# sarpaykent/GotenNet

Measured on AMD Instinct MI355X. Metric: molecules/sec (energy+force forward), rMD17 aspirin batch=128, 1/2/4/8 MI355X, higher is better.
Workload: dtype f32 (2xfp16-split MFMA with block exponents, fp32 accumulate); 1 GPU; rmd17_aspirin batch=128/GPU (N=2688 atoms, E=54368 edges incl. self-loops), n_atom_basis=256, n_interactions=6, lmax=2, n_rbf=32, heads=8, sep_dir/sep_tensor, energy+forces; global_batch=128, parallelism=dp1 (molecule shards, 1 all-reduce)

## Files before the change

gotennet_amd/csrc/gn_backward.hip:

```cpp
#include "gn_common.h"
#include "gn_tune.h"
#include "gn_sh.h"
#include "gn_highl.h"

namespace gn {


template <int K>
__device__ __forceinline__ void slot_sums(const float (&v)[K], int lps, int lp, float* __restrict__ arr, size_t base) {
    constexpr int KP = K <= 4 ? 4 : (K <= 8 ? 8 : (K <= 16 ? 16 : 32));
    if (lps >= KP) {
        float vals[KP];
#pragma unroll
        for (int k = 0; k < KP; ++k) vals[k] = k < K ? v[k] : 0.f;
        multi_group_sum<KP>(vals, lps, lp);
        const int stride = lps / KP;
        if ((lp & (stride - 1)) == 0 && lp / stride < K) arr[base + lp / stride] = vals[0];
    } else {
#pragma unroll
        for (int k = 0; k < K; ++k) {
            const float s = group_sum(v[k], lps);
            if (lp == 0) arr[base + k] = s;
        }
    }
}

template <int MS>
__device__ __forceinline__ void slot_head_sums(const float* hrow, int lps, int lp, int H, float* __restrict__ out) {
    const int rpl = lps / H, hh = lp / rpl, part = lp - hh * rpl;
    const float* hp = hrow + hh * (MS * rpl) + part * MS;
    float hv = hp[0];
#pragma unroll
    for (int k = 1; k < MS; ++k) hv += hp[k];
    hv = group_sum(hv, rpl);
    if (part == 0) out[hh] = hv;
}

constexpr int GS_CAP = 2048;
template <bool GS_LDS>
struct HeadGrads {
    float* gsl; float* g_s; int e0, H;
    __device__ __forceinline__ float& operator()(int e, int h) const {
        if constexpr (GS_LDS) return gsl[(e - e0) * H + h];
        else return g_s[(size_t)e * H + h];
    }
    __device__ __forceinline__ void copy_out(int e1) const {
        if constexpr (GS_LDS) {
            const int n = (e1 - e0) * H;
            for (int idx = threadIdx.x; idx < n; idx += 256) g_s[(size_t)e0 * H + idx] = gsl[idx];
        }
    }
};
template <typename Grads>
__device__ __forceinline__ void softmax_bwd_head(int e0, int e1, int H, int h, float dot, const float* __restrict__ a,
                                                 const float* __restrict__ a_soft, const int* __restrict__ outdeg,
                                                 const int* __restrict__ src, float inv_sqrt_f, Grads GS) {
    for (int e = e0 + (threadIdx.x & 63); e < e1; e += 64) {
        const float nrm = outdeg ? sqrtf((float)outdeg[src[e]]) * inv_sqrt_f : inv_sqrt_f;
        const float av = a[(size_t)e * H + h];
        const float sv = a_soft ? a_soft[(size_t)e * H + h] : av;
        GS(e, h) = av * GS(e, h) - (sv / nrm) * dot;
    }
}
__device__ __forceinline__ void score_bwd_edge(float gs, float4 qi, float4 kj, float4 pta, float4& gq, float* __restrict__ g_pta) {
    float4 a_ta, d_ta;
    act_pair4(pta, GN_ACT_SILU, a_ta, d_ta);
    gq = fma4(gs, kj * a_ta, gq);
    st4_nt(g_pta, ((qi * kj) * gs) * d_ta);
}
__device__ __forceinline__ float4 score_bwd_edge_k(float gs, float4 qi, float4 pta, float4 gk) {
    return fma4(gs, qi * act4(pta, GN_ACT_SILU), gk);
}

template <int LMAX, int FC = 0>
__global__ __launch_bounds__(256) GN_WPE(GN_W_HTR_SRC) void htr_bwd_source_kernel(
    const float* __restrict__ gtp, const float* __restrict__ pre_t,
    const float* __restrict__ EQ, const float* __restrict__ EK, const float* __restrict__ rl,
    const int* __restrict__ colptr, const int* __restrict__ perm, const int* __restrict__ dst, int N, int F_rt,
    float* __restrict__ gEK) {
    constexpr int act = GN_ACT_SILU;
    constexpr int D = (LMAX + 1) * (LMAX + 1) - 1;
    constexpr int CH = D < 9 ? D : 9;
    __shared__ __attribute__((aligned(16))) float red[CH * 1024];
    const int F = FC ? FC : F_rt;
    const int j = xcd_item(blockIdx.x, N);
    if (j < 0) return;
    GN_SLOT_GEOMETRY(FC);
    const int p0 = colptr[j], p1 = colptr[j + 1];
    float4 ek[D], acc[D];
#pragma unroll
    for (int m = 0; m < D; ++m) { ek[m] = ld4(EK + ((size_t)j * D + m) * F + c0); acc[m] = zero4(); }
    for (int pp = p0 + slot; pp < p1; pp += ns) {
        const int e = perm[pp];
        const float4 gw = ld4(gtp + (size_t)e * F + c0) * act4(ld4(pre_t + (size_t)e * F + c0), act);
        const float* qi = EQ + (size_t)dst[pp] * D * F + c0;
        const float* re = rl + (size_t)e * D;
        int m0 = 0;
#pragma unroll
        for (int l = 1; l <= LMAX; ++l) {
            float4 eq[2 * LMAX + 1];
            float r[2 * LMAX + 1];
            float4 pa = zero4();
            float rr = 0.f;
#pragma unroll
            for (int mm = 0; mm < 2 * l + 1; ++mm) {
                eq[mm] = ld4(qi + (size_t)(m0 + mm) * F);
                r[mm] = re[m0 + mm];
                pa = fma4(r[mm], eq[mm], pa);
                rr = fmaf(r[mm], r[mm], rr);
            }
            const float4 v = gw * pa * (rr - 2.0f);
#pragma unroll
            for (int mm = 0; mm < 2 * l + 1; ++mm)
                acc[m0 + mm] = fma4(r[mm], v, fma4(gw, eq[mm], acc[m0 + mm]));
            m0 += 2 * l + 1;
        }
    }
    reduce_rows<D>(acc, red, slot, c0, F, ns, [&](int row, float4 s) { st4(gEK + ((size_t)j * D + row) * F + c0, s); });
}

template <int LMAX, bool SEP_DIR, bool SEP_TENSOR>
struct MsgShape {
    static constexpr int D = (LMAX + 1) * (LMAX + 1) - 1;
    static constexpr int ND = SEP_DIR ? LMAX : 1;
    static constexpr int NT = SEP_TENSOR ? LMAX : 1;
    static constexpr int M = 1 + ND + NT;
    __host__ __device__ static constexpr bool is_dir(int b) { return b >= 1 && b < 1 + ND; }
    __host__ __device__ static constexpr int lo(int b) { return is_dir(b) ? (SEP_DIR ? b : 1) : (SEP_TENSOR ? b - ND : 1); }
    __host__ __device__ static constexpr int hi(int b) { return is_dir(b) ? (SEP_DIR ? b : LMAX) : (SEP_TENSOR ? b - ND : LMAX); }
    __host__ __device__ static constexpr int first_row(int l) { return l * l - 1; }
};


template <int LMAX, bool SEP_DIR, bool SEP_TENSOR, bool GS_LDS, bool FIRST, int FC>
__device__ __forceinline__ void msg_bwd_target_body(const MsgBwdArgs& p, float* gsl, float* red, float* hsum, const float* __restrict__ x_, const float* __restrict__ v_, const float* __restrict__ eproj_, const float* __restrict__ a_, const float* __restrict__ qk_, const float* __restrict__ X_in_, const float* __restrict__ rl_, const float* __restrict__ cut_, const int* __restrict__ outdeg_, const float* __restrict__ g_h1_, const float* __restrict__ g_X1_, const int* __restrict__ rowptr_, const int* __restrict__ src_, float* __restrict__ g_eproj_, float* __restrict__ g_s_, float* __restrict__ g_nproj_, float* __restrict__ g_rl_, float* __restrict__ g_cut_) {
    using S = MsgShape<LMAX, SEP_DIR, SEP_TENSOR>;
    constexpr int D = S::D, M = S::M;
    const int N = p.N, F = FC ? FC : p.F, H = p.H;
    const int i = xcd_item(blockIdx.x, N);
    if (i < 0) return;
    GN_SLOT_GEOMETRY(FC);
    const int e0 = rowptr_[i], e1 = rowptr_[i + 1];
    const int per_head = (M * F) / H;
    int hb[M];
// ... 293 lines not shown
        if (row < MB) st4(g_x + (size_t)j * ldxv + row * F + c0, sv);
        else if (row < 2 * MB) st4(g_v + (size_t)j * ldxv + (row - MB) * F + c0, sv);
        else {
            const size_t off = ((size_t)j * D + (row - 2 * MB)) * F + c0;
            st4(g_X_out + off, ld4(g_X1 + off) + sv);
        }
    });
    if (FIRST)
        for (int b = MB + slot; b < M; b += ns) {
            st4(g_x + (size_t)j * ldxv + b * F + c0, zero4());
            st4(g_v + (size_t)j * ldxv + b * F + c0, zero4());
        }
}
#define GN_MSGB_SOURCE_PTRS(p)                                                                                        \
    p.x, p.v, p.ldxv, p.X_in, p.eproj, p.lde, p.a, p.rl, p.cut, p.g_h1, p.g_X1, p.dst, p.colptr, p.perm, p.g_eproj, p.g_x, p.g_v, \
        p.g_X_out, p.g_rl
template <int LMAX, bool SEP_DIR, bool SEP_TENSOR, int FC = 0>
__global__ __launch_bounds__(256) GN_WPE(GN_W_MSG_MRG) void msg_bwd_merged_kernel(const MsgBwdArgs p, float* __restrict__ ga) {
    msg_bwd_merged_body<LMAX, SEP_DIR, SEP_TENSOR, FC, false>(GN_MSGB_SOURCE_PTRS(p), p.g_cut, ga, p.N, p.F, p.H);
}
template <int LMAX, bool SEP_DIR, bool SEP_TENSOR, int FC = 0>
__global__ __launch_bounds__(256) GN_WPE(GN_W_MSG_MRG_F) void msg_bwd_merged_first_kernel(const MsgBwdArgs p, float* __restrict__ ga) {
    msg_bwd_merged_body<LMAX, SEP_DIR, SEP_TENSOR, FC, true>(GN_MSGB_SOURCE_PTRS(p), p.g_cut, ga, p.N, p.F, p.H);
}

template <int FC = 0>
__global__ __launch_bounds__(256) void msg_bwd_gk_kernel(const MsgBwdArgs p) {
    __shared__ __attribute__((aligned(16))) float red[1024];
    const int N = p.N, F = FC ? FC : p.F, H = p.H;
    const int j = xcd_item(blockIdx.x, N);
    if (j < 0) return;
    GN_SLOT_GEOMETRY(FC);
    const int hq = c0 / (F / H);
    float4 gk[1] = {zero4()};
    for (int pp = p.colptr[j] + slot; pp < p.colptr[j + 1]; pp += ns) {
        const int e = p.perm[pp], i = p.dst[pp];
        gk[0] = score_bwd_edge_k(p.g_s[(size_t)e * H + hq], ld4(p.qk + (size_t)i * p.ldqk + c0),
                                 ld4_nt(p.eproj + (size_t)e * p.lde + c0), gk[0]);
    }
    reduce_rows<1>(gk, red, slot, c0, F, ns, [&](int, float4 sv) { st4(p.g_nproj + (size_t)j * p.ldn + F + c0, sv); });
}

template <bool GS_LDS, int FC>
__device__ __forceinline__ void attn_bwd_body(const MsgBwdArgs& p, const float* __restrict__ ga_parts, int G, size_t gstride,
                                              float* red, float* gsl, int i) {
    const int F = FC ? FC : p.F, H = p.H;
    GN_SLOT_GEOMETRY(FC);
    const int e0 = p.rowptr[i], e1 = p.rowptr[i + 1];
    const HeadGrads<GS_LDS> GS{gsl, p.g_s, e0, H};
    {
        const int wave = threadIdx.x >> 6, lane = threadIdx.x & 63;
        for (int h = wave; h < H; h += 4) {
            float dot = 0.f;
            for (int e = e0 + lane; e < e1; e += 64) {
                float ga = 0.f;
                for (int q = 0; q < G; ++q) ga += ga_parts[q * gstride + (size_t)e * H + h];
                GS(e, h) = ga;
                dot += p.a[(size_t)e * H + h] * ga;
            }
            softmax_bwd_head(e0, e1, H, h, wave_sum(dot), p.a, p.a_soft, p.outdeg, p.src, p.inv_sqrt_f, GS);
        }
    }
    __syncthreads();
    GS.copy_out(e1);
    const int hq = c0 / (F / H);
    const float4 qi = ld4(p.qk + (size_t)i * p.ldqk + c0);
    float4 gq = zero4();
    for (int e = e0 + slot; e < e1; e += ns) {
        const float4 kj = ld4(p.qk + (size_t)p.src[e] * p.ldqk + F + c0);
        score_bwd_edge(GS(e, hq), qi, kj, ld4_nt(p.eproj + (size_t)e * p.lde + c0), gq, p.g_eproj + (size_t)e * p.lde + c0);
    }
    st4(&red[slot * F + c0], gq);
    __syncthreads();
    if (slot == 0) st4(p.g_nproj + (size_t)i * p.ldn + c0, red4(red, c0, F, ns));
}
template <int FC = 0>
__global__ __launch_bounds__(256) void attn_bwd_kernel(const MsgBwdArgs p, const float* __restrict__ ga_parts, int G, size_t gstride) {
    __shared__ __attribute__((aligned(16))) float red[1024];
    __shared__ float gsl[GS_CAP];
    const int i = xcd_item(blockIdx.x, p.N);
    if (i < 0) return;
    if ((p.rowptr[i + 1] - p.rowptr[i]) * p.H <= GS_CAP) attn_bwd_body<true, FC>(p, ga_parts, G, gstride, red, gsl, i);
    else attn_bwd_body<false, FC>(p, ga_parts, G, gstride, red, gsl, i);
}

template <int LMAX, int LLO, int LHI, bool SCALAR, int FC>
__device__ __forceinline__ void msg_bwd_merged_group_body(
    const float* __restrict__ x, const float* __restrict__ v, int ldxv, const float* __restrict__ X_in,
    const float* __restrict__ eproj, int lde, const float* __restrict__ a, const float* __restrict__ rl,
    const float* __restrict__ cut, const float* __restrict__ g_h1, const float* __restrict__ g_X1,
    const int* __restrict__ dst, const int* __restrict__ colptr, const int* __restrict__ perm,
    float* __restrict__ g_eproj, float* __restrict__ g_x, float* __restrict__ g_v, float* __restrict__ g_X_out,
    float* __restrict__ g_rl, float* __restrict__ ga_slice, float* __restrict__ cut_slice, int N, int F_rt, int H) {
    constexpr int D = (LMAX + 1) * (LMAX + 1) - 1;
    constexpr int M = 1 + 2 * LMAX;
    constexpr int NL = LHI - LLO + 1;
    constexpr int XR = (LHI + 1) * (LHI + 1) - LLO * LLO, M0 = LLO * LLO - 1;
    constexpr int NB = (SCALAR ? 1 : 0) + 2 * NL;
    constexpr int ROWS = 2 * NB + XR;
    constexpr int CH = ROWS < 9 ? ROWS : 9;
    constexpr int KP = (XR + 8) <= 16 ? 16 : 32;
    __shared__ __attribute__((aligned(16))) float red[CH * 1024];
    __shared__ __attribute__((aligned(16))) float own[ROWS * 256];
    const int F = FC ? FC : F_rt;
    const int j = xcd_item(blockIdx.x, N);
    if (j < 0) return;
    GN_SLOT_GEOMETRY(FC);
    const int p0 = colptr[j], p1 = colptr[j + 1];
    const int per_head = (M * F) / H;
    auto vblock = [&](int k) { return SCALAR ? (k == 0 ? 0 : (k <= NL ? LLO + k - 1 : LMAX + LLO + k - 1 - NL))
                                             : (k < NL ? LLO + k : LMAX + LLO + k - NL); };
    for (int idx = threadIdx.x * 4; idx < ROWS * F; idx += 1024) {
        const int r = idx / F, c = idx - r * F;
        const float* g = r < NB ? x + (size_t)j * ldxv + vblock(r) * F
                                : (r < 2 * NB ? v + (size_t)j * ldxv + vblock(r - NB) * F
                                              : X_in + ((size_t)j * D + M0 + (r - 2 * NB)) * F);
        st4(own + idx, ld4(g + c));
    }
    float4 acc[ROWS];
#pragma unroll
    for (int r = 0; r < ROWS; ++r) acc[r] = zero4();
    __syncthreads();

    int pp = p0 + slot;
    int e_n = 0, i_n = 0;
    if (pp < p1) { e_n = perm[pp]; i_n = dst[pp]; }
    for (; pp < p1; pp += ns) {
        const int e = e_n, i = i_n;
        if (pp + ns < p1) { e_n = perm[pp + ns]; i_n = dst[pp + ns]; }
        const float* tr = eproj + (size_t)e * lde + F + c0;
        float* gtr = g_eproj + (size_t)e * lde + F + c0;
        const float* ar = a + (size_t)e * H;
        const float* re = rl + (size_t)e * D;
        const float* gXi = g_X1 + (size_t)i * D * F + c0;
        int oc = c0;
        asm volatile("" : "+v"(oc));
        const float* ox = own + oc;
        const float* ov = own + NB * F + oc;
        const float* oX = own + 2 * NB * F + oc;
        float4 tf[NB], gxa[XR];
        float ab_[NB];
#pragma unroll
        for (int k = 0; k < NB; ++k) tf[k] = ld4_nt(tr + vblock(k) * F);
#pragma unroll
        for (int m = 0; m < XR; ++m) gxa[m] = ld4(gXi + (size_t)(M0 + m) * F);
        float4 gh = zero4();
        if (SCALAR) gh = ld4(g_h1 + (size_t)i * F + c0);
        const float ce = cut[e];
#pragma unroll
        for (int k = 0; k < NB; ++k) ab_[k] = ar[(vblock(k) * F + c0) / per_head];
        float cutp = 0.f;
        float vals[KP];
#pragma unroll
        for (int k = 0; k < KP; ++k) vals[k] = 0.f;
        auto block = [&](int b, int k, float4 go) {
            const float4 tfb = tf[k], xb = ld4(ox + k * F), vb = ld4(ov + k * F);
            const int hb = (b * F + c0) / per_head;
            const float ab = ab_[k];
            st4_nt(gtr + b * F, (go * xb) * ce);
            cutp += hsum4(go * tfb * xb);
            const float pa = hsum4(go * vb);
#pragma unroll
            for (int h = 0; h < 8; ++h) vals[XR + h] += (hb == h) ? pa : 0.f;
            acc[k] = fma4(go, tfb * ce, acc[k]);
            acc[NB + k] = fma4(ab, go, acc[NB + k]);
            return fma4(ab, vb, (tfb * xb) * ce);
// ... 431 lines not shown
        for (int n = n0 + lane; n < n1; n += 64) s += y[n];
        s = wave_sum(s);
        if (lane == 0) energy[b] = ((mean && n1 > n0) ? s / (float)(n1 - n0) : s) + mol_shift;
    }
    if (atom_scale)
        for (int n = n0 + (int)threadIdx.x; n < n1; n += 1024) atom_scale[n] = mean ? 1.0f / (float)(n1 - n0) : 1.0f;
}

__global__ void head_grad_kernel(const float* __restrict__ pre1, const float* __restrict__ W2, float scale,
                                 const float* __restrict__ atom_scale, int N, int Hd, float* __restrict__ gpre1, int act) {
    const size_t idx = (size_t)blockIdx.x * blockDim.x + threadIdx.x;
    if (idx >= (size_t)N * Hd) return;
    const float sc = atom_scale ? scale * atom_scale[idx / Hd] : scale;
    gpre1[idx] = sc * W2[idx % Hd] * dact1(pre1[idx], act);
}

}

static bool bwd_dim_ok_wide(int F) { return F >= 16 && F <= 1024 && gn::is_pow2(F); }

#define GN_SWITCH_LMAX(KERNEL, grid, block, st, ...)                                                   \
    switch (lmax) {                                                                                    \
        case 1: hipLaunchKernelGGL(gn::KERNEL<1>, grid, block, 0, st, __VA_ARGS__); break;             \
        case 2: hipLaunchKernelGGL(gn::KERNEL<2>, grid, block, 0, st, __VA_ARGS__); break;             \
        case 3: hipLaunchKernelGGL(gn::KERNEL<3>, grid, block, 0, st, __VA_ARGS__); break;             \
        case 4: hipLaunchKernelGGL(gn::KERNEL<4>, grid, block, 0, st, __VA_ARGS__); break;             \
        case 5: hipLaunchKernelGGL(gn::KERNEL<5>, grid, block, 0, st, __VA_ARGS__); break;             \
        case 6: hipLaunchKernelGGL(gn::KERNEL<6>, grid, block, 0, st, __VA_ARGS__); break;             \
        case 7: hipLaunchKernelGGL(gn::KERNEL<7>, grid, block, 0, st, __VA_ARGS__); break;             \
        default: hipLaunchKernelGGL(gn::KERNEL<8>, grid, block, 0, st, __VA_ARGS__); break;            \
    }

template <int FC>
static void htr_backward_launch(const float* g_t_out, const float* pre_t, const float* w, const float* EQ, const float* EK,
                                const float* rl, const int* rowptr, const int* src, const int* dst, const int* colptr,
                                const int* perm, int N, int F, int lmax, float* gEQ, float* gEK, float* g_rl, float* g_pre_t,
                                hipStream_t st) {
    const dim3 grid(gn::xcd_grid(N)), block(256);
#define GN_HTRB_T(L, LLO, LHI, FIRST)                                                                            \
    hipLaunchKernelGGL((gn::htr_bwd_target_group_kernel<L, LLO, LHI, FIRST, FC>), grid, block, 0, st, g_t_out, pre_t, w, \
                       EQ, EK, rl, rowptr, src, N, F, gEQ, g_rl, g_pre_t)
#define GN_HTRB_S(...)                                                                                           \
    hipLaunchKernelGGL((gn::__VA_ARGS__), grid, block, 0, st, g_t_out, pre_t, EQ, EK, rl, colptr, perm, dst, N, F, gEK)
    switch (lmax) {
        case 1: GN_HTRB_T(1, 1, 1, true); GN_HTRB_S(htr_bwd_source_kernel<1, FC>); break;
        case 2: GN_HTRB_T(2, 1, 2, true); GN_HTRB_S(htr_bwd_source_kernel<2, FC>); break;
        case 3: GN_HTRB_T(3, 1, 3, true); GN_HTRB_S(htr_bwd_source_group_kernel<3, 1, 3, FC>); break;
        default: GN_HTRB_T(4, 1, 2, true); GN_HTRB_T(4, 3, 4, false); GN_HTRB_S(htr_bwd_source_group_kernel<4, 1, 4, FC>); break;
    }
#undef GN_HTRB_T
#undef GN_HTRB_S
}

extern "C" int gn_htr_backward(const float* g_t_out, const float* pre_t, const float* w, const float* w_raw,
                               const float* EQ,
                               const float* EK, const float* rl, const int* rowptr, const int* src, const int* dst,
                               const int* colptr, const int* perm, int N, int F, int lmax_arg, int mode,
                               float* gEQ, float* gEK, float* g_rl, float* g_pre_t, int act, void* stream) {
    const int lmax = lmax_arg & 0xff;
    if ((lmax_arg & ~(0xff | GN_LMAX_SLICED)) || !bwd_dim_ok_wide(F) || N < 0 || lmax < 1 || lmax > 8 || mode < 0 || mode > 31 ||
        act < 0 || act >= GN_ACT_COUNT)
        return GN_ERR_BAD_ARG;
    if (N == 0) return GN_OK;
    hipStream_t st = (hipStream_t)stream;
    if (gn_use_highl(lmax_arg) || F > 256 || (!mode && act != GN_ACT_SILU))
        return gn_highl_htr_backward(g_t_out, pre_t, w, w_raw, EQ, EK, rl, rowptr, src, dst, colptr, perm, N, F, lmax,
                                     mode, gEQ, gEK, g_rl, g_pre_t, act, st);
    if (mode)
        return gn_htr_backward_general(g_t_out, pre_t, w, w_raw, EQ, EK, rl, rowptr, src, dst, colptr, perm, N, F, lmax,
                                       mode, gEQ, gEK, g_rl, g_pre_t, act, st);
    if (F == 256) htr_backward_launch<256>(g_t_out, pre_t, w, EQ, EK, rl, rowptr, src, dst, colptr, perm, N, F, lmax, gEQ, gEK, g_rl, g_pre_t, st);
    else htr_backward_launch<0>(g_t_out, pre_t, w, EQ, EK, rl, rowptr, src, dst, colptr, perm, N, F, lmax, gEQ, gEK, g_rl, g_pre_t, st);
    GN_LAUNCH_CHECK();
    return GN_OK;
}

template <int L, int LLO, int LHI, bool SC, int FC>
static inline void gn_launch_msg_bwd_group(dim3 grid, dim3 block, hipStream_t st, const gn::MsgBwdArgs& p, float* ga_slice, float* cut_slice) {
    if constexpr (LLO == 3 && LHI == 3)
        hipLaunchKernelGGL((gn::msg_bwd_merged_group3_kernel<L, LLO, LHI, SC, FC>), grid, block, 0, st, p, ga_slice, cut_slice);
    else
        hipLaunchKernelGGL((gn::msg_bwd_merged_group_kernel<L, LLO, LHI, SC, FC>), grid, block, 0, st, p, ga_slice, cut_slice);
}
template <int L, bool SD, bool ST, int FC>
static void gn_launch_msg_bwd(dim3 grid, dim3 block, hipStream_t st, const gn::MsgBwdArgs& p, float* ga_parts) {
    constexpr bool GROUPED = L >= 3 && SD && ST;
    if (ga_parts != nullptr) {
        if (!p.X_in) hipLaunchKernelGGL((gn::msg_bwd_merged_first_kernel<L, SD, ST, FC>), grid, block, 0, st, p, ga_parts);
        else if constexpr (!GROUPED) hipLaunchKernelGGL((gn::msg_bwd_merged_kernel<L, SD, ST, FC>), grid, block, 0, st, p, ga_parts);
        hipLaunchKernelGGL(gn::attn_bwd_kernel<FC>, grid, block, 0, st, p, ga_parts, 1, (size_t)0);
        hipLaunchKernelGGL(gn::msg_bwd_gk_kernel<FC>, grid, block, 0, st, p);
    } else if (!p.X_in) {
        hipLaunchKernelGGL((gn::msg_bwd_target_kernel<L, SD, ST, true, FC>), grid, block, 0, st, p);
        hipLaunchKernelGGL((gn::msg_bwd_source_kernel<L, SD, ST, true, FC>), grid, block, 0, st, p);
    } else if constexpr (!GROUPED) {
        hipLaunchKernelGGL((gn::msg_bwd_target_kernel<L, SD, ST>), grid, block, 0, st, p);
        hipLaunchKernelGGL((gn::msg_bwd_source_kernel<L, SD, ST>), grid, block, 0, st, p);
    }
}

extern "C" int gn_message_backward_groups(int lmax_arg, int sep_dir, int sep_tensor, int act) {
    const int lmax = lmax_arg & 0xff;
    if (gn_use_highl(lmax_arg) || act != GN_ACT_SILU) return 1;
    return (lmax >= 3 && sep_dir && sep_tensor) ? lmax - 1 : 1;
}

template <int FC>
static void message_backward_launch(const gn::MsgBwdArgs& p, int lmax, int sep_dir, int sep_tensor, bool groups, float* ga_parts,
                                    long E, hipStream_t st) {
    const dim3 grid(gn::xcd_grid(p.N)), block(256);
    if (groups) {
        const size_t gs = (size_t)E * p.H;
#define GN_MSGB_M(L, LLO, LHI, SC, G)                                                                        \
    gn_launch_msg_bwd_group<L, LLO, LHI, SC, FC>(grid, block, st, p, ga_parts + (size_t)(G) * gs, p.g_cut + (size_t)(G) * E)
        if (lmax == 3) { GN_MSGB_M(3, 1, 2, true, 0); GN_MSGB_M(3, 3, 3, false, 1); }
        else { GN_MSGB_M(4, 1, 2, true, 0); GN_MSGB_M(4, 3, 3, false, 1); GN_MSGB_M(4, 4, 4, false, 2); }
#undef GN_MSGB_M
        hipLaunchKernelGGL(gn::attn_bwd_kernel<FC>, grid, block, 0, st, p, ga_parts, lmax - 1, gs);
        hipLaunchKernelGGL(gn::msg_bwd_gk_kernel<FC>, grid, block, 0, st, p);
        return;
    }
#define GN_MSGB_CASE(L, SD, ST, W) \
    case (L) * 4 + (SD ? 2 : 0) + (ST ? 1 : 0): gn_launch_msg_bwd<L, SD, ST, W>(grid, block, st, p, ga_parts); break
    switch (lmax * 4 + (sep_dir ? 2 : 0) + (sep_tensor ? 1 : 0)) {
        case 4: case 5: case 6: case 7:
            gn_launch_msg_bwd<1, false, false, FC>(grid, block, st, p, ga_parts);
            break;
        GN_MSGB_CASE(2, false, false, 0);
        GN_MSGB_CASE(2, false, true, 0);
        GN_MSGB_CASE(2, true, false, 0);
        GN_MSGB_CASE(2, true, true, FC);
        GN_MSGB_CASE(3, false, false, 0);
        GN_MSGB_CASE(3, false, true, 0);
        GN_MSGB_CASE(3, true, false, 0);
        GN_MSGB_CASE(3, true, true, FC);
        GN_MSGB_CASE(4, false, false, 0);
        GN_MSGB_CASE(4, false, true, 0);
        GN_MSGB_CASE(4, true, false, 0);
        default: gn_launch_msg_bwd<4, true, true, FC>(grid, block, st, p, ga_parts); break;
    }
#undef GN_MSGB_CASE
}

static int message_backward(
    const float* x, const float* v, int ldxv, const float* eproj, int lde, const float* a,
    const float* qk, int ldqk, const float* X_in, const float* rl, const float* cut, const int* outdeg,
    const float* g_h1, const float* g_X1,
    const int* rowptr, const int* src, const int* dst, const int* colptr, const int* perm,
    float* g_eproj, float* g_s, float* g_nproj, int ldn, float* g_x, float* g_v, float* g_X_out,
    float* g_rl, float* g_cut, float* ga_parts, long E,
    int N, int F, int H, int lmax_arg, int sep_dir, int sep_tensor, int act, void* stream, const float* a_soft) {
    const int lmax = lmax_arg & 0xff;
    const bool amax = (lmax_arg & GN_LMAX_MAX) != 0;
    if (amax && ((lmax_arg & GN_LMAX_MEAN) || !ga_parts || !X_in)) return GN_ERR_BAD_ARG;
    if ((lmax_arg & ~(0xff | GN_LMAX_SLICED | GN_LMAX_MEAN | GN_LMAX_MAX)) || !bwd_dim_ok_wide(F) || N < 0 || H <= 0 || !gn::is_pow2(H) || (F / 4) % H || (F / 4) / H > 64 || lmax < 1 || lmax > 8 ||
        (ldxv & 3) || (lde & 3) || (ldqk & 3) || (ldn & 3) || g_X_out == g_X1 || act < 0 || act >= GN_ACT_COUNT)
        return GN_ERR_BAD_ARG;
    if (!X_in && (act != GN_ACT_SILU || gn_use_highl(lmax_arg) || F > 256)) return GN_ERR_BAD_ARG;
    if (N == 0) return GN_OK;
    gn::MsgBwdArgs p{x, v, ldxv, eproj, lde, a, qk, ldqk, X_in, rl, cut, outdeg, g_h1, g_X1,
                     rowptr, src, dst, colptr, perm, g_eproj, g_s, g_nproj, ldn, g_x, g_v, g_X_out, g_rl, g_cut,
                     N, F, H, (float)(1.0 / sqrt((double)F)), act, (lmax_arg & GN_LMAX_MEAN) ? 1 : 0, amax ? ga_parts : nullptr, a_soft};
    hipStream_t st = (hipStream_t)stream;
    if (gn_use_highl(lmax_arg) || F > 256 || act != GN_ACT_SILU) return gn_highl_message_backward(p, lmax, sep_dir, sep_tensor, st);
    const int G = gn_message_backward_groups(lmax_arg, sep_dir, sep_tensor, act);
    const bool groups = X_in && G > 1;
    if (groups && (ga_parts == nullptr || E <= 0)) return GN_ERR_BAD_ARG;
    if (groups && H > 8) {
        hipError_t err = hipMemsetAsync(g_cut + E, 0, (size_t)(G - 1) * (size_t)E * sizeof(float), st);
        if (err != hipSuccess) return (int)err;
        return gn_highl_message_backward(p, lmax, sep_dir, sep_tensor, st);
    }
    if (F == 256) message_backward_launch<256>(p, lmax, sep_dir, sep_tensor, groups, ga_parts, E, st);
    else message_backward_launch<0>(p, lmax, sep_dir, sep_tensor, groups, ga_parts, E, st);
    GN_LAUNCH_CHECK();
    return GN_OK;
}

extern "C" int gn_message_backward(
    const float* x, const float* v, int ldxv, const float* eproj, int lde, const float* a,
    const float* qk, int ldqk, const float* X_in, const float* rl, const float* cut, const int* outdeg,
    const float* g_h1, const float* g_X1,
    const int* rowptr, const int* src, const int* dst, const int* colptr, const int* perm,
    float* g_eproj, float* g_s, float* g_nproj, int ldn, float* g_x, float* g_v, float* g_X_out,
    float* g_rl, float* g_cut, float* ga_parts, long E,
    int N, int F, int H, int lmax_arg, int sep_dir, int sep_tensor, int act, void* stream) {
    return message_backward(x, v, ldxv, eproj, lde, a, qk, ldqk, X_in, rl, cut, outdeg, g_h1, g_X1, rowptr, src, dst, colptr,
                            perm, g_eproj, g_s, g_nproj, ldn, g_x, g_v, g_X_out, g_rl, g_cut, ga_parts, E, N, F, H, lmax_arg,
                            sep_dir, sep_tensor, act, stream, nullptr);
}

extern "C" int gn_message_backward_dropout(
    const float* x, const float* v, int ldxv, const float* eproj, int lde, const float* a, const float* a_soft,
    const float* qk, int ldqk, const float* X_in, const float* rl, const float* cut, const int* outdeg,
    const float* g_h1, const float* g_X1,
    const int* rowptr, const int* src, const int* dst, const int* colptr, const int* perm,
    float* g_eproj, float* g_s, float* g_nproj, int ldn, float* g_x, float* g_v, float* g_X_out,
    float* g_rl, float* g_cut, float* ga_parts, long E,
    int N, int F, int H, int lmax_arg, int sep_dir, int sep_tensor, int act, void* stream) {
    if (!a_soft) return GN_ERR_BAD_ARG;
    return message_backward(x, v, ldxv, eproj, lde, a, qk, ldqk, X_in, rl, cut, outdeg, g_h1, g_X1, rowptr, src, dst, colptr,
                            perm, g_eproj, g_s, g_nproj, ldn, g_x, g_v, g_X_out, g_rl, g_cut, ga_parts, E, N, F, H, lmax_arg,
// ... 137 lines not shown
```

gotennet_amd/csrc/gn_tune.h:

```cpp
#pragma once

#define GN_WPE_ATTR(n) __attribute__((amdgpu_waves_per_eu(n, n)))

#ifndef GN_W_K6
#define GN_W_K6 3
#endif
#ifndef GN_W_K6_G
#define GN_W_K6_G 3
#endif
#ifndef GN_W_MSG_TGT
#define GN_W_MSG_TGT 0
#endif
#ifndef GN_W_MSG_SRC
#define GN_W_MSG_SRC 2
#endif
#ifndef GN_W_HTR_TGT
#define GN_W_HTR_TGT 0
#endif
#ifndef GN_W_HTR_SRC
#define GN_W_HTR_SRC 0
#endif
#ifndef GN_W_HTR_SRC_G
#define GN_W_HTR_SRC_G 0
#endif
#ifndef GN_W_HTR_EDGE
#define GN_W_HTR_EDGE 0
#endif
#ifndef GN_W_ATTN
#define GN_W_ATTN 0
#endif

#ifndef GN_K6_MERGE34
#define GN_K6_MERGE34 1
#endif
#ifndef GN_W_K6_G34
#define GN_W_K6_G34 2
#endif
#ifndef GN_K6G_CH
#define GN_K6G_CH 16
#endif

#ifndef GN_W_MSG_MRG_G
#define GN_W_MSG_MRG_G 2
#endif
#ifndef GN_W_MSG_MRG_G3
#define GN_W_MSG_MRG_G3 3
#endif
#ifndef GN_W_MSG_MRG
#define GN_W_MSG_MRG 0
#endif
#ifndef GN_W_MSG_MRG_F
#define GN_W_MSG_MRG_F 2
#endif
#ifndef GN_MSGB_PF3
#define GN_MSGB_PF3 4
#endif

#ifndef GN_GEMM_BIG_MIN
#define GN_GEMM_BIG_MIN 900
#endif
#ifndef GN_GEMM_BIG_CAP
#define GN_GEMM_BIG_CAP 512
#endif
#ifndef GN_SPLIT_MINW
#define GN_SPLIT_MINW 2
#endif
#ifndef GN_GEMM_NT_MB
#define GN_GEMM_NT_MB 100.0
#endif
#ifndef GN_GEMM_NT_LO
#define GN_GEMM_NT_LO (-1)
#endif
#ifndef GN_GEMM_PANEL_MAX
#define GN_GEMM_PANEL_MAX 2048
#endif
#ifndef GN_F16_SMALL_WIDE
#define GN_F16_SMALL_WIDE 1
#endif
#ifndef GN_F16_MID_ROWS
#define GN_F16_MID_ROWS 30000
#endif
#ifndef GN_F16_MID_CAP
#define GN_F16_MID_CAP 768
#endif
#ifndef GN_F16_SMALL_CAP
#define GN_F16_SMALL_CAP 1024
#endif
#ifndef GN_HTR_CLOSED
#define GN_HTR_CLOSED 1
#endif
#ifndef GN_HTR_CLOSED_ALL
#define GN_HTR_CLOSED_ALL 4
#endif
#ifndef GN_ATTN_WAVE
#define GN_ATTN_WAVE 1
#endif

#define GN_TUNE_CAT_(a, b) a##b
#define GN_TUNE_CAT(a, b) GN_TUNE_CAT_(a, b)
#define GN_WPE_SEL_0
#define GN_WPE_SEL_1 GN_WPE_ATTR(1)
#define GN_WPE_SEL_2 GN_WPE_ATTR(2)
#define GN_WPE_SEL_3 GN_WPE_ATTR(3)
#define GN_WPE_SEL_4 GN_WPE_ATTR(4)
#define GN_WPE_SEL_5 GN_WPE_ATTR(5)
#define GN_WPE_SEL_6 GN_WPE_ATTR(6)
#define GN_WPE_SEL_8 GN_WPE_ATTR(8)
#define GN_WPE(n) GN_TUNE_CAT(GN_WPE_SEL_, n)
```

Before: 23030 molecules/s.

## Add wave-per-node attention backward kernel with head-vectorized softmax and prefetched edge loads

Adds a wave-per-node variant of the attention-score backward kernel. Each 64-lane wave handles one destination node, packing four nodes into a 256-thread block. Per-edge head gradients are kept in a per-wave LDS strip, head rows are read as float4, and neighbor key and edge-projection loads are software-prefetched in groups of 8. A matching wave-per-node gk kernel is added, but the default GN_MSGB_WAVE=2 enables only the attention variant. The change is meant to remove block-level syncs, shared reductions and idle threads on low-degree nodes, at the cost of more registers and a dependence on F==256.

Measured after the change: 23110 molecules/s, median of 6. No clear change (+0.4%).

```diff
diff --git a/gotennet_amd/csrc/gn_backward.hip b/gotennet_amd/csrc/gn_backward.hip
--- a/gotennet_amd/csrc/gn_backward.hip
+++ b/gotennet_amd/csrc/gn_backward.hip
@@ -51,15 +51,19 @@
         }
     }
 };
+__device__ __forceinline__ float softmax_bwd_nrm(const int* __restrict__ outdeg, const int* __restrict__ src, int e, float inv_sqrt_f) {
+    return outdeg ? sqrtf((float)outdeg[src[e]]) * inv_sqrt_f : inv_sqrt_f;
+}
+__device__ __forceinline__ float softmax_bwd_elem(float av, float sv, float nrm, float ga, float dot) { return av * ga - (sv / nrm) * dot; }
 template <typename Grads>
 __device__ __forceinline__ void softmax_bwd_head(int e0, int e1, int H, int h, float dot, const float* __restrict__ a,
                                                  const float* __restrict__ a_soft, const int* __restrict__ outdeg,
                                                  const int* __restrict__ src, float inv_sqrt_f, Grads GS) {
     for (int e = e0 + (threadIdx.x & 63); e < e1; e += 64) {
-        const float nrm = outdeg ? sqrtf((float)outdeg[src[e]]) * inv_sqrt_f : inv_sqrt_f;
+        const float nrm = softmax_bwd_nrm(outdeg, src, e, inv_sqrt_f);
         const float av = a[(size_t)e * H + h];
         const float sv = a_soft ? a_soft[(size_t)e * H + h] : av;
-        GS(e, h) = av * GS(e, h) - (sv / nrm) * dot;
+        GS(e, h) = softmax_bwd_elem(av, sv, nrm, GS(e, h), dot);
     }
 }
 __device__ __forceinline__ void score_bwd_edge(float gs, float4 qi, float4 kj, float4 pta, float4& gq, float* __restrict__ g_pta) {
@@ -519,6 +523,181 @@
     if (i < 0) return;
     if ((p.rowptr[i + 1] - p.rowptr[i]) * p.H <= GS_CAP) attn_bwd_body<true, FC>(p, ga_parts, G, gstride, red, gsl, i);
     else attn_bwd_body<false, FC>(p, ga_parts, G, gstride, red, gsl, i);
+}
+
+constexpr int MSGB_W_STRIP = 512;
+constexpr int MSGB_W_U = 8;
+
+template <bool GS_LDS, int FC, int HC, bool HFIX>
+__device__ __forceinline__ void attn_bwd_wave_body(
+    const float* __restrict__ a, const float* __restrict__ a_soft, const int* __restrict__ outdeg, const int* __restrict__ src,
+    const float* __restrict__ qk, int ldqk, const float* __restrict__ eproj, float* __restrict__ g_eproj, int lde,
+    const float* ga_parts, int G, size_t gstride, float* g_s, float* __restrict__ g_nproj, int ldn, float inv_sqrt_f, int H_rt,
+    int i, int e0, int e1, float* strip) {
+    static_assert(FC == 256 && HC % 4 == 0 && (HC || !HFIX), "a row is one wave; head rows are read as float4");
+    constexpr int F = FC, U = MSGB_W_U;
+    const int H = HFIX ? HC : H_rt;
+    const int lane = threadIdx.x & 63, c0 = lane * 4;
+    const HeadGrads<GS_LDS> GS{strip, g_s, e0, H};
+    int jj[U];
+    float4 kj[U], pta[U];
+    auto indices = [&](int eb) {
+#pragma unroll
+        for (int u = 0; u < U; ++u) jj[u] = src[eb + u < e1 ? eb + u : e1 - 1];
+    };
+    auto request = [&](int eb) {
+#pragma unroll
+        for (int u = 0; u < U; ++u) {
+            kj[u] = ld4(qk + (size_t)jj[u] * ldqk + F + c0);
+            pta[u] = ld4_nt(eproj + (size_t)(eb + u < e1 ? eb + u : e1 - 1) * lde + c0);
+        }
+    };
+    if (e1 > e0) {
+        indices(e0);
+        request(e0);
+        if (e0 + U < e1) indices(e0 + U);
+    }
+    if constexpr (HC == 0) {
+        for (int h = 0; h < H; ++h) {
+            float dot = 0.f;
+            for (int e = e0 + lane; e < e1; e += 64) {
+                float ga = 0.f;
+                for (int q = 0; q < G; ++q) ga += ga_parts[q * gstride + (size_t)e * H + h];
+                GS(e, h) = ga;
+                dot += a[(size_t)e * H + h] * ga;
+            }
+            softmax_bwd_head(e0, e1, H, h, wave_sum(dot), a, a_soft, outdeg, src, inv_sqrt_f, GS);
+        }
+    } else if (e1 > e0) {
+        constexpr int HH = HC ? HC : 4;
+        const int last = e0 + ((e1 - e0 - 1) & ~63);
+        for (int hb = 0; hb < H; hb += HH) {
+            float av[HH], sv[HH], dot[HH], nrm = 0.f;
+#pragma unroll
+            for (int h = 0; h < HH; ++h) dot[h] = 0.f;
+            auto row = [&](int e) {
+                nrm = softmax_bwd_nrm(outdeg, src, e, inv_sqrt_f);
+#pragma unroll
+                for (int k = 0; k < HH; k += 4) {
+                    const float4 t = ld4(a + (size_t)e * H + hb + k);
+                    const float4 s = a_soft ? ld4(a_soft + (size_t)e * H + hb + k) : t;
+                    av[k] = t.x; av[k + 1] = t.y; av[k + 2] = t.z; av[k + 3] = t.w;
+                    sv[k] = s.x; sv[k + 1] = s.y; sv[k + 2] = s.z; sv[k + 3] = s.w;
+                }
+            };
+            auto finish = [&](int e) {
+#pragma unroll
+                for (int h = 0; h < HH; ++h) GS(e, hb + h) = softmax_bwd_elem(av[h], sv[h], nrm, GS(e, hb + h), dot[h]);
+            };
+            for (int e = e0 + lane; e < e1; e += 64) {
+                row(e);
+                float ga[HH];
+#pragma unroll
+                for (int h = 0; h < HH; ++h) ga[h] = 0.f;
+                for (int q = 0; q < G; ++q)
+#pragma unroll
+                    for (int k = 0; k < HH; k += 4) {
+                        const float4 t = ld4(ga_parts + q * gstride + (size_t)e * H + hb + k);
+                        ga[k] += t.x; ga[k + 1] += t.y; ga[k + 2] += t.z; ga[k + 3] += t.w;
+                    }
+#pragma unroll
+                for (int h = 0; h < HH; ++h) {
+                    GS(e, hb + h) = ga[h];
+                    dot[h] += av[h] * ga[h];
+                }
+            }
+#pragma unroll
+            for (int h = 0; h < HH; ++h) dot[h] = wave_sum(dot[h]);
+            if (last + lane < e1) finish(last + lane);
+            for (int e = e0 + lane; e < last; e += 64) {
+                row(e);
+                finish(e);
+            }
+        }
+    }
+    if constexpr (!GS_LDS) __builtin_amdgcn_s_waitcnt(0);
+    __builtin_amdgcn_wave_barrier();
+    if constexpr (GS_LDS) {
+        const int n = (e1 - e0) * H;
+        for (int idx = lane; idx < n; idx += 64) g_s[(size_t)e0 * H + idx] = strip[idx];
+    }
+    const int hq = c0 / (F / H);
+    const float4 qi = ld4(qk + (size_t)i * ldqk + c0);
+    float4 gq[4] = {zero4(), zero4(), zero4(), zero4()};
+    for (int eb = e0; eb < e1; eb += U) {
+        if (eb != e0) {
+            request(eb);
+            if (eb + U < e1) indices(eb + U);
+        }
+#pragma unroll
+        for (int u = 0; u < U; ++u)
+            if (eb + u < e1) score_bwd_edge(GS(eb + u, hq), qi, kj[u], pta[u], gq[u & 3], g_eproj + (size_t)(eb + u) * lde + c0);
+    }
+    st4(g_nproj + (size_t)i * ldn + c0, ((gq[0] + gq[1]) + gq[2]) + gq[3]);
+}
+template <int FC, int HC, bool HFIX>
+__global__ __launch_bounds__(256) void attn_bwd_wave_kernel(const MsgBwdArgs p, const float* ga_parts, int G, size_t gstride) {
+    __shared__ float strips[4 * MSGB_W_STRIP];
+    const int grp = xcd_item(blockIdx.x, (p.N + 3) >> 2);
+    if (grp < 0) return;
+    const int wave = __builtin_amdgcn_readfirstlane((int)(threadIdx.x >> 6));
+    const int i = 4 * grp + wave;
+    if (i >= p.N) return;
+    const int e0 = p.rowptr[i], e1 = p.rowptr[i + 1];
+    float* strip = strips + wave * MSGB_W_STRIP;
+    if ((e1 - e0) * p.H <= MSGB_W_STRIP)
+        attn_bwd_wave_body<true, FC, HC, HFIX>(p.a, p.a_soft, p.outdeg, p.src, p.qk, p.ldqk, p.eproj, p.g_eproj, p.lde, ga_parts, G, gstride,
+                                         p.g_s, p.g_nproj, p.ldn, p.inv_sqrt_f, p.H, i, e0, e1, strip);
+    else
+        attn_bwd_wave_body<false, FC, HC, HFIX>(p.a, p.a_soft, p.outdeg, p.src, p.qk, p.ldqk, p.eproj, p.g_eproj, p.lde, ga_parts, G, gstride,
+                                          p.g_s, p.g_nproj, p.ldn, p.inv_sqrt_f, p.H, i, e0, e1, strip);
+}
+
+template <int FC>
+__device__ __forceinline__ void msg_bwd_gk_wave_body(
+    const float* __restrict__ g_s, const float* __restrict__ qk, int ldqk, const float* __restrict__ eproj, int lde,
+    const int* __restrict__ perm, const int* __restrict__ dst, float* __restrict__ g_nproj, int ldn, int H, int j, int p0, int p1) {
+    static_assert(FC == 256, "a row is one wave");
+    constexpr int F = FC, U = MSGB_W_U;
+    const int lane = threadIdx.x & 63, c0 = lane * 4;
+    const int hq = c0 / (F / H);
+    float4 gk[4] = {zero4(), zero4(), zero4(), zero4()};
+    int ee[U], ii[U];
+    auto indices = [&](int pb) {
+#pragma unroll
+        for (int u = 0; u < U; ++u) {
+            const int pp = pb + u < p1 ? pb + u : p1 - 1;
+            ee[u] = perm[pp];
+            ii[u] = dst[pp];
+        }
+    };
+    if (p1 > p0) indices(p0);
+    for (int pb = p0; pb < p1; pb += U) {
+        float gs[U];
+        float4 qi[U], pta[U];
+#pragma unroll
+        for (int u = 0; u < U; ++u) {
+            gs[u] = g_s[(size_t)ee[u] * H + hq];
+            qi[u] = ld4(qk + (size_t)ii[u] * ldqk + c0);
+            pta[u] = ld4_nt(eproj + (size_t)ee[u] * lde + c0);
+        }
+        if (pb + U < p1) indices(pb + U);
+#pragma unroll
+        for (int u = 0; u < U; ++u) {
+            const float4 t = score_bwd_edge_k(gs[u], qi[u], pta[u], gk[u & 3]);
+            const bool live = pb + u < p1;
+            gk[u & 3] = make_float4(live ? t.x : gk[u & 3].x, live ? t.y : gk[u & 3].y, live ? t.z : gk[u & 3].z, live ? t.w : gk[u & 3].w);
+        }
+    }
+    st4(g_nproj + (size_t)j * ldn + F + c0, ((gk[0] + gk[1]) + gk[2]) + gk[3]);
+}
+template <int FC>
+__global__ __launch_bounds__(256) void msg_bwd_gk_wave_kernel(const MsgBwdArgs p) {
+    const int grp = xcd_item(blockIdx.x, (p.N + 3) >> 2);
+    if (grp < 0) return;
+    const int j = 4 * grp + __builtin_amdgcn_readfirstlane((int)(threadIdx.x >> 6));
+    if (j >= p.N) return;
+    msg_bwd_gk_wave_body<FC>(p.g_s, p.qk, p.ldqk, p.eproj, p.lde, p.perm, p.dst, p.g_nproj, p.ldn, p.H, j, p.colptr[j], p.colptr[j + 1]);
 }
 
 template <int LMAX, int LLO, int LHI, bool SCALAR, int FC>
@@ -1116,14 +1295,25 @@
     else
         hipLaunchKernelGGL((gn::msg_bwd_merged_group_kernel<L, LLO, LHI, SC, FC>), grid, block, 0, st, p, ga_slice, cut_slice);
 }
+template <int FC>
+static void gn_launch_attn_bwd_gk(dim3 grid, dim3 block, hipStream_t st, const gn::MsgBwdArgs& p, const float* ga_parts, int G, size_t gstride) {
+    const bool wave = p.F == 256 && 64 % p.H == 0;
+    const dim3 wgrid(gn::xcd_grid((p.N + 3) / 4));
+    if (GN_MSGB_WAVE_ATTN && wave && p.H == 8) hipLaunchKernelGGL((gn::attn_bwd_wave_kernel<256, 8, true>), wgrid, block, 0, st, p, ga_parts, G, gstride);
+    else if (GN_MSGB_WAVE_ATTN && wave && p.H % 8 == 0) hipLaunchKernelGGL((gn::attn_bwd_wave_kernel<256, 8, false>), wgrid, block, 0, st, p, ga_parts, G, gstride);
+    else if (GN_MSGB_WAVE_ATTN && wave && p.H == 4) hipLaunchKernelGGL((gn::attn_bwd_wave_kernel<256, 4, true>), wgrid, block, 0, st, p, ga_parts, G, gstride);
+    else if (GN_MSGB_WAVE_ATTN && wave) hipLaunchKernelGGL((gn::attn_bwd_wave_kernel<256, 0, false>), wgrid, block, 0, st, p, ga_parts, G, gstride);
+    else hipLaunchKernelGGL(gn::attn_bwd_kernel<FC>, grid, block, 0, st, p, ga_parts, G, gstride);
+    if (GN_MSGB_WAVE_GK && wave) hipLaunchKernelGGL(gn::msg_bwd_gk_wave_kernel<256>, wgrid, block, 0, st, p);
+    else hipLaunchKernelGGL(gn::msg_bwd_gk_kernel<FC>, grid, block, 0, st, p);
+}
 template <int L, bool SD, bool ST, int FC>
 static void gn_launch_msg_bwd(dim3 grid, dim3 block, hipStream_t st, const gn::MsgBwdArgs& p, float* ga_parts) {
     constexpr bool GROUPED = L >= 3 && SD && ST;
     if (ga_parts != nullptr) {
         if (!p.X_in) hipLaunchKernelGGL((gn::msg_bwd_merged_first_kernel<L, SD, ST, FC>), grid, block, 0, st, p, ga_parts);
         else if constexpr (!GROUPED) hipLaunchKernelGGL((gn::msg_bwd_merged_kernel<L, SD, ST, FC>), grid, block, 0, st, p, ga_parts);
-        hipLaunchKernelGGL(gn::attn_bwd_kernel<FC>, grid, block, 0, st, p, ga_parts, 1, (size_t)0);
-        hipLaunchKernelGGL(gn::msg_bwd_gk_kernel<FC>, grid, block, 0, st, p);
+        gn_launch_attn_bwd_gk<FC>(grid, block, st, p, ga_parts, 1, (size_t)0);
     } else if (!p.X_in) {
         hipLaunchKernelGGL((gn::msg_bwd_target_kernel<L, SD, ST, true, FC>), grid, block, 0, st, p);
         hipLaunchKernelGGL((gn::msg_bwd_source_kernel<L, SD, ST, true, FC>), grid, block, 0, st, p);
@@ -1150,8 +1340,7 @@
         if (lmax == 3) { GN_MSGB_M(3, 1, 2, true, 0); GN_MSGB_M(3, 3, 3, false, 1); }
         else { GN_MSGB_M(4, 1, 2, true, 0); GN_MSGB_M(4, 3, 3, false, 1); GN_MSGB_M(4, 4, 4, false, 2); }
 #undef GN_MSGB_M
-        hipLaunchKernelGGL(gn::attn_bwd_kernel<FC>, grid, block, 0, st, p, ga_parts, lmax - 1, gs);
-        hipLaunchKernelGGL(gn::msg_bwd_gk_kernel<FC>, grid, block, 0, st, p);
+        gn_launch_attn_bwd_gk<FC>(grid, block, st, p, ga_parts, lmax - 1, gs);
         return;
     }
 #define GN_MSGB_CASE(L, SD, ST, W) \
diff --git a/gotennet_amd/csrc/gn_tune.h b/gotennet_amd/csrc/gn_tune.h
--- a/gotennet_amd/csrc/gn_tune.h
+++ b/gotennet_amd/csrc/gn_tune.h
@@ -95,6 +95,11 @@
 #ifndef GN_ATTN_WAVE
 #define GN_ATTN_WAVE 1
 #endif
+#ifndef GN_MSGB_WAVE
+#define GN_MSGB_WAVE 2
+#endif
+#define GN_MSGB_WAVE_ATTN (GN_MSGB_WAVE == 1 || GN_MSGB_WAVE == 2)
+#define GN_MSGB_WAVE_GK (GN_MSGB_WAVE == 1 || GN_MSGB_WAVE == 3)
 
 #define GN_TUNE_CAT_(a, b) a##b
 #define GN_TUNE_CAT(a, b) GN_TUNE_CAT_(a, b)
```
